# Jackie-Chou/MC-CNN-python

Measured on AMD Instinct MI355X. Metric: Mdisparities/s (HxWxD / s) end-to-end match.py timed region, images resident in HBM, higher is better.
Workload: dtype f32; 1 GPU; cfg2: 750x500 synthetic stereo pair, D=256, one pair per GPU; weights=converted reference checkpoint

## Files before the change

### mc-cnn-python_amd/csrc/cost_volume.hip

```cpp
#include "common.h"

namespace mccnn {

constexpr int CV_TW = 64;
constexpr int CV_DT = 64;
constexpr int CV_C = 64;
#ifndef CVM_WAVES_PER_SIMD
#define CVM_WAVES_PER_SIMD 6
#endif
constexpr int CV_LD = 68;

template <bool PIXEL_MAJOR>
__global__ __launch_bounds__(256) void cost_volume_exact_kernel(const float *__restrict__ fl,
                                                                const float *__restrict__ fr, int H, int W, int D,
                                                                float *__restrict__ lcv, float *__restrict__ rcv, int Dp)
{
    __shared__ __attribute__((aligned(16))) float sR[(CV_TW + CV_DT - 1) * CV_LD];
    __shared__ __attribute__((aligned(16))) float sL[CV_TW * CV_LD];
    const int w0 = blockIdx.x * CV_TW, h = blockIdx.y, d0 = blockIdx.z * CV_DT;
    if (w0 + CV_TW - 1 < d0) return;
    const int tid = threadIdx.x;
    const size_t rowbase = (size_t)h * W;
    for (int i = tid; i < CV_TW * 16; i += 256) {
        const int px = i >> 4, c4 = i & 15;
        float4 v = make_float4(0.f, 0.f, 0.f, 0.f);
        if (w0 + px < W) v = *reinterpret_cast<const float4 *>(fl + (rowbase + w0 + px) * CV_C + c4 * 4);
        *reinterpret_cast<float4 *>(&sL[px * CV_LD + c4 * 4]) = v;
    }
    const int xr0 = w0 - d0 - (CV_DT - 1);
    for (int i = tid; i < (CV_TW + CV_DT - 1) * 16; i += 256) {
        const int r = i >> 4, c4 = i & 15;
        const int x = xr0 + r;
        float4 v = make_float4(0.f, 0.f, 0.f, 0.f);
        if (x >= 0 && x < W) v = *reinterpret_cast<const float4 *>(fr + (rowbase + x) * CV_C + c4 * 4);
        *reinterpret_cast<float4 *>(&sR[r * CV_LD + c4 * 4]) = v;
    }
    __syncthreads();

    const int wl = tid & 63, dq = tid >> 6;
    const int w = w0 + wl;
    float a[CV_C];
#pragma unroll
    for (int c4 = 0; c4 < 16; ++c4) {
        const float4 v = *reinterpret_cast<const float4 *>(&sL[wl * CV_LD + c4 * 4]);
        a[c4 * 4 + 0] = v.x; a[c4 * 4 + 1] = v.y; a[c4 * 4 + 2] = v.z; a[c4 * 4 + 3] = v.w;
    }
    const size_t plane = (size_t)H * W;
    constexpr int TP = 65;
    float *const sT = sL;
    if (PIXEL_MAJOR) __syncthreads();
    for (int k = 0; k < 16; ++k) {
        const int d = d0 + dq * 16 + k;
        if (d >= D) break;
        const int r = wl + (CV_DT - 1) - (dq * 16 + k);
        if (w < W && w >= d) {
            const float *b = &sR[r * CV_LD];
            float acc[8];
#pragma unroll
            for (int i = 0; i < 8; ++i) {
                const float4 b0 = *reinterpret_cast<const float4 *>(b + i * 8);
                const float4 b1 = *reinterpret_cast<const float4 *>(b + i * 8 + 4);
                const float p0 = a[i * 8 + 0] * b0.x, p1 = a[i * 8 + 1] * b0.y, p2 = a[i * 8 + 2] * b0.z,
                            p3 = a[i * 8 + 3] * b0.w, p4 = a[i * 8 + 4] * b1.x, p5 = a[i * 8 + 5] * b1.y,
                            p6 = a[i * 8 + 6] * b1.z, p7 = a[i * 8 + 7] * b1.w;
                if (i == 0) {
                    acc[0] = p0; acc[1] = p1; acc[2] = p2; acc[3] = p3;
                    acc[4] = p4; acc[5] = p5; acc[6] = p6; acc[7] = p7;
                } else {
                    acc[0] += p0; acc[1] += p1; acc[2] += p2; acc[3] += p3;
                    acc[4] += p4; acc[5] += p5; acc[6] += p6; acc[7] += p7;
                }
            }
            float s = ((acc[0] + acc[1]) + (acc[2] + acc[3])) + ((acc[4] + acc[5]) + (acc[6] + acc[7]));
            s = 0.f + s;
            s = -1.f * s;
            if (PIXEL_MAJOR) {
                sT[wl * TP + dq * 16 + k] = s;
            } else {
                lcv[(size_t)d * plane + rowbase + w] = s;
                rcv[(size_t)d * plane + rowbase + (w - d)] = s;
            }
        }
    }
    if (PIXEL_MAJOR) {
        __syncthreads();
        const int nd = min(CV_DT, D - d0);
        const int dl = tid & 63;
        for (int px = tid >> 6; px < CV_TW; px += 4) {
            const int ww = w0 + px, d = d0 + dl;
            if (ww < W && dl < nd && ww >= d) lcv[(rowbase + ww) * (size_t)Dp + d] = sT[px * TP + dl];
        }
        for (int xi = tid >> 6; xi < CV_TW + CV_DT - 1; xi += 4) {
            const int x = xr0 + xi, d = d0 + dl, px = x + d - w0;
            if (x >= 0 && dl < nd && px >= 0 && px < CV_TW && w0 + px < W)
                rcv[(rowbase + x) * (size_t)Dp + d] = sT[px * TP + dl];
        }
    }
}

constexpr int CVP_TW = 63;
#ifndef CVP_ABL
#define CVP_ABL 0
#endif
__device__ __forceinline__ bool cvp_never(int D) { return D == 12345; }
__global__ __launch_bounds__(256, 3) void cost_volume_exact_pairs_kernel(const float *__restrict__ fl,
                                                                         const float *__restrict__ fr, int H, int W, int D,
                                                                         float *__restrict__ lcv, float *__restrict__ rcv,
                                                                         int Dp)
{
    constexpr int RING = 128;
    __shared__ __attribute__((aligned(16))) float sR[RING * CV_LD];
    __shared__ __attribute__((aligned(16))) float sL[CV_TW * CV_LD];
    const int w0 = (int)blockIdx.x * CVP_TW - 1, h = blockIdx.y;
    const int tid = threadIdx.x;
    const size_t rowbase = (size_t)h * W;
    for (int i = tid; i < CV_TW * 16; i += 256) {
        const int px = i >> 4, c4 = i & 15;
        float4 v = make_float4(0.f, 0.f, 0.f, 0.f);
        if (w0 + px >= 0 && w0 + px < W) v = *reinterpret_cast<const float4 *>(fl + (rowbase + w0 + px) * CV_C + c4 * 4);
        *reinterpret_cast<float4 *>(&sL[px * CV_LD + c4 * 4]) = v;
    }
    for (int i = tid; i < (CV_TW + CV_DT - 1) * 16; i += 256) {
        const int x = w0 - (CV_DT - 1) + (i >> 4), c4 = i & 15;
        float4 v = make_float4(0.f, 0.f, 0.f, 0.f);
        if (x >= 0 && x < W) v = *reinterpret_cast<const float4 *>(fr + (rowbase + x) * CV_C + c4 * 4);
        *reinterpret_cast<float4 *>(&sR[(x & (RING - 1)) * CV_LD + c4 * 4]) = v;
    }
    __syncthreads();

    const int wl = tid & 63, dq = tid >> 6;
    const int w = w0 + wl;
    float a[CV_C];
#pragma unroll
    for (int c4 = 0; c4 < 16; ++c4) {
        const float4 v = *reinterpret_cast<const float4 *>(&sL[wl * CV_LD + c4 * 4]);
        a[c4 * 4 + 0] = v.x; a[c4 * 4 + 1] = v.y; a[c4 * 4 + 2] = v.z; a[c4 * 4 + 3] = v.w;
    }
    constexpr int TP = CV_LD;
    float *const sT = sL;
    __syncthreads();
#pragma unroll 1
    for (int d0 = 0; d0 < D && w0 + CV_TW - 1 >= d0; d0 += CV_DT) {
        const bool more = d0 + CV_DT < D && w0 + CV_TW - 1 >= d0 + CV_DT;
        float4 nx[4];
#pragma unroll
        for (int q = 0; q < 4; ++q) {
            const int i = tid + q * 256, x = w0 - d0 - (2 * CV_DT - 1) + (i >> 4), c4 = i & 15;
            nx[q] = make_float4(0.f, 0.f, 0.f, 0.f);
            if (more && x >= 0 && x < W) nx[q] = *reinterpret_cast<const float4 *>(fr + (rowbase + x) * CV_C + c4 * 4);
        }
#pragma unroll 1
        for (int kk = 0; kk < (((CVP_ABL & 1) && !cvp_never(D)) ? 0 : 8); ++kk) {
            const int dloc = dq * 16 + 2 * kk;
            const int r = (w - d0 - dloc) & (RING - 1);
            const float *b = &sR[r * CV_LD];
            float acc[8], acn[8];
            float4 n0 = *reinterpret_cast<const float4 *>(b), n1 = *reinterpret_cast<const float4 *>(b + 4);
#pragma unroll
            for (int i = 0; i < 8; ++i) {
                const float bv[8] = {n0.x, n0.y, n0.z, n0.w, n1.x, n1.y, n1.z, n1.w};
                if (i < 7) {
                    n0 = *reinterpret_cast<const float4 *>(b + (i + 1) * 8);
                    n1 = *reinterpret_cast<const float4 *>(b + (i + 1) * 8 + 4);
                }
#pragma unroll
                for (int j = 0; j < 8; j += 4) {
                    if (i == 0) {
                        asm volatile("v_mul_f32 %0, %8, %12\n\tv_mul_f32 %1, %9, %13\n\tv_mul_f32 %2, %10, %14\n\tv_mul_f32 %3, %11, %15\n\t"
                                     "v_mul_f32_dpp %4, %12, %8 wave_shr:1 row_mask:0xf bank_mask:0xf bound_ctrl:1\n\t"
                                     "v_mul_f32_dpp %5, %13, %9 wave_shr:1 row_mask:0xf bank_mask:0xf bound_ctrl:1\n\t"
                                     "v_mul_f32_dpp %6, %14, %10 wave_shr:1 row_mask:0xf bank_mask:0xf bound_ctrl:1\n\t"
                                     "v_mul_f32_dpp %7, %15, %11 wave_shr:1 row_mask:0xf bank_mask:0xf bound_ctrl:1"
                                     : "=&v"(acc[j]), "=&v"(acc[j + 1]), "=&v"(acc[j + 2]), "=&v"(acc[j + 3]),
                                       "=&v"(acn[j]), "=&v"(acn[j + 1]), "=&v"(acn[j + 2]), "=&v"(acn[j + 3])
                                     : "v"(a[j]), "v"(a[j + 1]), "v"(a[j + 2]), "v"(a[j + 3]),
                                       "v"(bv[j]), "v"(bv[j + 1]), "v"(bv[j + 2]), "v"(bv[j + 3]));
                    } else {
                        float t0, t1, t2, t3;
                        asm volatile("v_mul_f32 %8, %12, %16\n\tv_mul_f32 %9, %13, %17\n\tv_mul_f32 %10, %14, %18\n\tv_mul_f32 %11, %15, %19\n\t"
                                     "v_add_f32 %0, %0, %8\n\tv_add_f32 %1, %1, %9\n\tv_add_f32 %2, %2, %10\n\tv_add_f32 %3, %3, %11\n\t"
                                     "v_mul_f32_dpp %8, %16, %12 wave_shr:1 row_mask:0xf bank_mask:0xf bound_ctrl:1\n\t"
                                     "v_mul_f32_dpp %9, %17, %13 wave_shr:1 row_mask:0xf bank_mask:0xf bound_ctrl:1\n\t"
                                     "v_mul_f32_dpp %10, %18, %14 wave_shr:1 row_mask:0xf bank_mask:0xf bound_ctrl:1\n\t"
                                     "v_mul_f32_dpp %11, %19, %15 wave_shr:1 row_mask:0xf bank_mask:0xf bound_ctrl:1\n\t"
                                     "v_add_f32 %4, %4, %8\n\tv_add_f32 %5, %5, %9\n\tv_add_f32 %6, %6, %10\n\tv_add_f32 %7, %7, %11"
                                     : "+v"(acc[j]), "+v"(acc[j + 1]), "+v"(acc[j + 2]), "+v"(acc[j + 3]),
                                       "+v"(acn[j]), "+v"(acn[j + 1]), "+v"(acn[j + 2]), "+v"(acn[j + 3]),
                                       "=&v"(t0), "=&v"(t1), "=&v"(t2), "=&v"(t3)
                                     : "v"(a[i * 8 + j]), "v"(a[i * 8 + j + 1]), "v"(a[i * 8 + j + 2]), "v"(a[i * 8 + j + 3]),
                                       "v"(bv[j]), "v"(bv[j + 1]), "v"(bv[j + 2]), "v"(bv[j + 3]));
                    }
                }
                __builtin_amdgcn_sched_barrier(0);
            }
            float s = ((acc[0] + acc[1]) + (acc[2] + acc[3])) + ((acc[4] + acc[5]) + (acc[6] + acc[7]));
            float sn = ((acn[0] + acn[1]) + (acn[2] + acn[3])) + ((acn[4] + acn[5]) + (acn[6] + acn[7]));
            s = 0.f + s;
            sn = 0.f + sn;
            s = -1.f * s;
            sn = -1.f * sn;
            const int d = d0 + dloc;
            if (wl >= 1 && w < W) {
                if (d < D && w >= d) sT[wl * TP + dloc] = s;
                if (d + 1 < D && w >= d + 1) sT[wl * TP + dloc + 1] = sn;
            }
        }
        __syncthreads();
#pragma unroll
        for (int q = 0; q < 4; ++q) {
            const int i = tid + q * 256, x = w0 - d0 - (2 * CV_DT - 1) + (i >> 4), c4 = i & 15;
            if (more) *reinterpret_cast<float4 *>(&sR[(x & (RING - 1)) * CV_LD + c4 * 4]) = nx[q];
        }
        const int nd = ((CVP_ABL & 2) && !cvp_never(D)) ? 0 : min(CV_DT, D - d0);
        const int xr0 = w0 - d0 - (CV_DT - 1);
        const int q4 = (tid & 15) * 4, sub = tid >> 4;
        for (int px = 1 + sub; px < CV_TW; px += 16) {
            const int ww = w0 + px, d = d0 + q4;
            if (ww >= W || q4 >= nd || ww < d) continue;
            const float4 v = *reinterpret_cast<const float4 *>(&sT[px * TP + q4]);
            float *dst = lcv + (rowbase + ww) * (size_t)Dp + d;
            if (q4 + 3 < nd && ww >= d + 3) {
                *reinterpret_cast<float4 *>(dst) = v;
            } else {
                const float e[4] = {v.x, v.y, v.z, v.w};
#pragma unroll
                for (int j = 0; j < 4; ++j)
                    if (q4 + j < nd && ww >= d + j) dst[j] = e[j];
            }
        }
        for (int xi = sub; xi < CV_TW + CV_DT - 1; xi += 16) {
            const int x = xr0 + xi, d = d0 + q4, px = x + d - w0;
            if (x < 0 || q4 >= nd || px + 3 < 1 || px >= CV_TW) continue;
            float *dst = rcv + (rowbase + x) * (size_t)Dp + d;
            if (q4 + 3 < nd && px >= 1 && px + 3 < CV_TW && w0 + px + 3 < W) {
                float4 v;
                v.x = sT[px * TP + q4];
                v.y = sT[(px + 1) * TP + q4 + 1];
                v.z = sT[(px + 2) * TP + q4 + 2];
                v.w = sT[(px + 3) * TP + q4 + 3];
                *reinterpret_cast<float4 *>(dst) = v;
            } else {
#pragma unroll
                for (int j = 0; j < 4; ++j)
                    if (q4 + j < nd && px + j >= 1 && px + j < CV_TW && w0 + px + j < W) dst[j] = sT[(px + j) * TP + q4 + j];
            }
        }
        __syncthreads();
    }
}

using f32x16 = __attribute__((ext_vector_type(16))) float;
typedef _Float16 cv_h8 __attribute__((ext_vector_type(8)));
typedef _Float16 cv_h4 __attribute__((ext_vector_type(4)));
constexpr int CVM_SP = 144;
constexpr int CVM_TP = 68;

__device__ __forceinline__ void cv_split4(const float4 v, cv_h4 &hi, cv_h4 &lo)
{
    const float x[4] = {__builtin_amdgcn_fmed3f(v.x * 1024.f, -65504.f, 65504.f),
                        __builtin_amdgcn_fmed3f(v.y * 1024.f, -65504.f, 65504.f),
                        __builtin_amdgcn_fmed3f(v.z * 1024.f, -65504.f, 65504.f),
                        __builtin_amdgcn_fmed3f(v.w * 1024.f, -65504.f, 65504.f)};
#pragma unroll
    for (int j = 0; j < 4; ++j) {
        const _Float16 h = (_Float16)x[j];
        hi[j] = h;
        lo[j] = (_Float16)(x[j] - (float)h);
    }
}

template <bool PIXEL_MAJOR>
__global__ __launch_bounds__(256, CVM_WAVES_PER_SIMD) void cost_volume_mfma_kernel(
    const float *__restrict__ fl, const float *__restrict__ fr, int H, int W, int D, float *__restrict__ lcv,
    float *__restrict__ rcv, int nwt, int nbands, int total, int Dp)
{
    constexpr int LDS_BYTES = (2 * 64 * CVM_SP > 64 * CVM_TP * 4) ? 2 * 64 * CVM_SP : 64 * CVM_TP * 4;
    __shared__ __attribute__((aligned(16))) char lds[LDS_BYTES];
    char *oL = lds, *oR = lds + 64 * CVM_SP;
    float *sT = reinterpret_cast<float *>(lds);
    int id;
    {
        const int b = blockIdx.x, qq = total >> 3, r = total & 7, xc = b & 7;
        id = (xc < r ? xc * (qq + 1) : r * (qq + 1) + (xc - r) * qq) + (b >> 3);
    }
    const int wt = id % nwt, band = (id / nwt) % nbands;
    const int h = id / (nwt * nbands);
    const int w0 = wt * 64;
    const int x0 = w0 - band * 64;
    if (x0 + 63 < 0) return;
    if (w0 - x0 - 63 >= D) return;
    const int tid = threadIdx.x;
    const size_t rowbase = (size_t)h * W;
    float4 vl[2][2], vr[2][2];
#pragma unroll
    for (int hf = 0; hf < 2; ++hf)
#pragma unroll
        for (int j = 0; j < 2; ++j) {
            const int p = j * 256 + tid, px = p >> 3, c4 = hf * 8 + (p & 7);
            vl[hf][j] = make_float4(0.f, 0.f, 0.f, 0.f);
            vr[hf][j] = make_float4(0.f, 0.f, 0.f, 0.f);
            if (w0 + px < W) vl[hf][j] = *reinterpret_cast<const float4 *>(fl + (rowbase + w0 + px) * CV_C + c4 * 4);
            const int x = x0 + px;
            if (x >= 0 && x < W) vr[hf][j] = *reinterpret_cast<const float4 *>(fr + (rowbase + x) * CV_C + c4 * 4);
        }
    const int wave = tid >> 6, lane = tid & 63;
    const int wr = (wave >> 1) * 32, wc = (wave & 1) * 32;
    f32x16 acc, acc2;
#pragma unroll
    for (int i = 0; i < 16; ++i) acc[i] = 0.f, acc2[i] = 0.f;
    const char *pa = oL + (wr + (lane & 31)) * CVM_SP + 16 * (lane >> 5);
    const char *pb = oR + (wc + (lane & 31)) * CVM_SP + 16 * (lane >> 5);
#pragma unroll
    for (int hf = 0; hf < 2; ++hf) {
        if (hf) __syncthreads();
#pragma unroll
        for (int j = 0; j < 2; ++j) {
            const int p = j * 256 + tid, px = p >> 3, c = p & 7;
            const int off = px * CVM_SP + (c >> 2) * 64 + (c & 3) * 8;
            cv_h4 hh, ll;
            cv_split4(vl[hf][j], hh, ll);
            *reinterpret_cast<cv_h4 *>(oL + off) = hh;
            *reinterpret_cast<cv_h4 *>(oL + off + 32) = ll;
            cv_split4(vr[hf][j], hh, ll);
            *reinterpret_cast<cv_h4 *>(oR + off) = hh;
            *reinterpret_cast<cv_h4 *>(oR + off + 32) = ll;
        }
        __syncthreads();
#pragma unroll
        for (int q = 0; q < 2; ++q) {
            const cv_h8 a_hi = *reinterpret_cast<const cv_h8 *>(pa + q * 64);
            const cv_h8 a_lo = *reinterpret_cast<const cv_h8 *>(pa + q * 64 + 32);
            const cv_h8 b_hi = *reinterpret_cast<const cv_h8 *>(pb + q * 64);
            const cv_h8 b_lo = *reinterpret_cast<const cv_h8 *>(pb + q * 64 + 32);
            acc2 = __builtin_amdgcn_mfma_f32_32x32x16_f16(a_lo, b_hi, acc2, 0, 0, 0);
            acc = __builtin_amdgcn_mfma_f32_32x32x16_f16(a_hi, b_hi, acc, 0, 0, 0);
            acc2 = __builtin_amdgcn_mfma_f32_32x32x16_f16(a_hi, b_lo, acc2, 0, 0, 0);
        }
    }
    __syncthreads();
    if (PIXEL_MAJOR) {
        constexpr int TP = 65;
#pragma unroll
        for (int rg = 0; rg < 16; ++rg) {
            const int row = wr + (rg & 3) + 8 * (rg >> 2) + 4 * (lane >> 5);
            const int col = wc + (lane & 31);
            sT[row * TP + col] = (acc[rg] + acc2[rg]) * (-1.f / 1048576.f);
        }
        __syncthreads();
        const int dbase = w0 - x0;
        for (int r = wave; r < 64; r += 4) {
            const int w = w0 + r, d = dbase + r - lane;
            if (w < W && d >= 0 && d < D && w >= d) lcv[(rowbase + w) * (size_t)Dp + d] = sT[r * TP + lane];
        }
        for (int c = wave; c < 64; c += 4) {
            const int x = x0 + c, d = dbase + lane - c;
            if (x >= 0 && w0 + lane < W && d >= 0 && d < D) rcv[(rowbase + x) * (size_t)Dp + d] = sT[lane * TP + c];
        }
        return;
    }
#pragma unroll
    for (int rg = 0; rg < 16; ++rg) {
        const int row = wr + (rg & 3) + 8 * (rg >> 2) + 4 * (lane >> 5);
        const int col = wc + (lane & 31);
        sT[((row - col) & 63) * CVM_TP + row] = (acc[rg] + acc2[rg]) * (-1.f / 1048576.f);
    }
    __syncthreads();
    const size_t plane = (size_t)H * W;
    const int dbase = w0 - x0;
    typedef float f4u __attribute__((ext_vector_type(4), aligned(4)));
    const int q = lane & 15, sub = lane >> 4;
    for (int rgp = wave; rgp < 16; rgp += 4) {
        const int row = rgp * 4 + sub;
        const int wl = 4 * q;
        const float4 t = *reinterpret_cast<const float4 *>(&sT[row * CVM_TP + wl]);
        const float v[4] = {t.x, t.y, t.z, t.w};
        const int w = w0 + wl;
        if (wl >= row || wl + 3 < row) {
            const int dd = wl >= row ? row : row - 64;
            const int d = dbase + dd;
            if (d < 0 || d >= D || w >= W) continue;
            float *pl = lcv + (size_t)d * plane + rowbase + w;
            float *pr = rcv + (size_t)d * plane + rowbase + (w - d);
            if (w + 3 < W) {
                f4u o;
                o[0] = v[0]; o[1] = v[1]; o[2] = v[2]; o[3] = v[3];
                *reinterpret_cast<f4u *>(pl) = o;
                *reinterpret_cast<f4u *>(pr) = o;
            } else {
#pragma unroll
                for (int j = 0; j < 4; ++j)
                    if (w + j < W) {
                        pl[j] = v[j];
                        pr[j] = v[j];
                    }
            }
        }
    }
    {
        const int row = tid >> 2, j = tid & 3;
        const int c = (row & ~3) + j;
        const int d = dbase + (c >= row ? row : row - 64);
        const int w = w0 + c;
        if ((row & 3) != 0 && d >= 0 && d < D && w < W) {
            const float v = sT[row * CVM_TP + c];
            lcv[(size_t)d * plane + rowbase + w] = v;
            rcv[(size_t)d * plane + rowbase + (w - d)] = v;
        }
    }
}

__global__ __launch_bounds__(64) void cost_volume_fill_kernel(float *__restrict__ lcv, float *__restrict__ rcv, int D,
                                                              int H, int W)
{
    __shared__ float tile[64 * 65];
    const int lane = threadIdx.x;
    const int d = D - 1 - blockIdx.y;
    const int h0 = blockIdx.x * 64;
    const int h = min(h0 + lane, H - 1);
    const int nrows = min(64, H - h0);
    if (blockIdx.z == 0) {
        float *L = lcv + ((size_t)d * H + h) * W;
        float x1 = L[d], x2 = L[d + 1], x3 = L[d + 2];
        for (int wtop = d - 1; wtop >= 0; wtop -= 64) {
            const int cnt = min(64, wtop + 1);
            for (int j = 0; j < cnt; ++j) {
                float s = 0.f - x1;
                s = s - x2;
                s = s - x3;
                const float v = -(s / 3.f);
                tile[lane * 65 + j] = v;
                x3 = x2; x2 = x1; x1 = v;
            }
            __syncthreads();
            if (lane < cnt)
                for (int r = 0; r < nrows; ++r)
                    lcv[((size_t)d * H + h0 + r) * W + (wtop - lane)] = tile[r * 65 + lane];
            __syncthreads();
        }
    } else {
        float *Rr = rcv + ((size_t)d * H + h) * W;
        float x1 = Rr[W - d - 3], x2 = Rr[W - d - 2], x3 = Rr[W - d - 1];
        for (int wbot = W - d; wbot < W; wbot += 64) {
            const int cnt = min(64, W - wbot);
            for (int j = 0; j < cnt; ++j) {
                float s = 0.f - x1;
                s = s - x2;
                s = s - x3;
                const float v = -(s / 3.f);
                tile[lane * 65 + j] = v;
                x1 = x2; x2 = x3; x3 = v;
            }
            __syncthreads();
            if (lane < cnt)
                for (int r = 0; r < nrows; ++r)
                    rcv[((size_t)d * H + h0 + r) * W + (wbot + lane)] = tile[r * 65 + lane];
            __syncthreads();
        }
    }
}

typedef uint32_t cv_u32x4 __attribute__((ext_vector_type(4)));
template <int NG>
__global__ __launch_bounds__(64) void cost_volume_fill_hwd_kernel(float *__restrict__ lcv, float *__restrict__ rcv, int D,
                                                                  int Dp, int H, int W)
{
    constexpr int PF = 8;
    constexpr int kDrop = 0x7ffffff0;
    const int lane = threadIdx.x, h = blockIdx.x;
    const bool left = blockIdx.y == 0;
    float *row = (left ? lcv : rcv) + (size_t)h * W * Dp;
    const __amdgpu_buffer_rsrc_t rs = __builtin_amdgcn_make_buffer_rsrc(row, 0, (int)((size_t)W * Dp * 4), 0x00020000);
    const unsigned pix = (unsigned)Dp * 4u;
    const int c_first = left ? D + 1 : max(W - D - 2, 0), nsteps = left ? D + 2 : W - c_first;
    auto col = [&](int t) { return left ? c_first - t : c_first + t; };
    int dbase[NG], voff[NG];
    float x1[NG][4], x2[NG][4], x3[NG][4];
#pragma unroll
    for (int g = 0; g < NG; ++g) {
        dbase[g] = g * 256 + lane * 4;
        voff[g] = dbase[g] < Dp ? dbase[g] * 4 : kDrop;
#pragma unroll
        for (int i = 0; i < 4; ++i) x1[g][i] = x2[g][i] = x3[g][i] = 0.f;
    }
    cv_u32x4 buf[PF][NG];
    auto issue = [&](int slot, int t) {
        const unsigned so = (unsigned)col(min(t, nsteps - 1)) * pix;
#pragma unroll
        for (int g = 0; g < NG; ++g) buf[slot][g] = __builtin_amdgcn_raw_buffer_load_b128(rs, voff[g], so, 0);
    };
#pragma unroll
    for (int k = 0; k < PF; ++k) issue(k, k);
    for (int t0 = 0; t0 < nsteps; t0 += PF) {
#pragma unroll
        for (int k = 0; k < PF; ++k) {
            const int t = t0 + k;
            if (t >= nsteps) continue;
            const int c = col(t);
#pragma unroll
            for (int g = 0; g < NG; ++g) {
                const cv_u32x4 u = buf[k][g];
                const float v[4] = {__uint_as_float(u.x), __uint_as_float(u.y), __uint_as_float(u.z), __uint_as_float(u.w)};
                cv_u32x4 o;
                bool any = false;
#pragma unroll
                for (int i = 0; i < 4; ++i) {
                    const int d = dbase[g] + i;
                    const bool stored = left ? c >= d : c < W - d;
                    float s = 0.f - x1[g][i];
                    s = s - x2[g][i];
                    s = s - x3[g][i];
                    const float val = stored ? v[i] : -(s / 3.f);
                    any |= !stored && d < D;
                    if (left) { x3[g][i] = x2[g][i]; x2[g][i] = x1[g][i]; x1[g][i] = val; }
                    else      { x1[g][i] = x2[g][i]; x2[g][i] = x3[g][i]; x3[g][i] = val; }
                    o[i] = __float_as_uint(val);
                }
                buffer_store_b128<0>(o, rs, any ? voff[g] : kDrop, (unsigned)c * pix);
            }
            issue(k, t + PF);
        }
    }
}


__global__ __launch_bounds__(64) void cost_volume_fill_hwd_lanes_kernel(float *__restrict__ lcv, float *__restrict__ rcv,
                                                                        int D, int Dp, int H, int W)
{
    constexpr int PF = 16;
    constexpr int kDrop = 0x7ffffff0;
    const int lane = threadIdx.x, h = blockIdx.x;
    const bool left = blockIdx.y == 0;
    const int d = (int)blockIdx.z * 64 + lane;
    const int dmax = min((int)blockIdx.z * 64 + 63, D - 1);
    if ((int)blockIdx.z * 64 >= D) return;
    float *row = (left ? lcv : rcv) + (size_t)h * W * Dp;
    const __amdgpu_buffer_rsrc_t rs = __builtin_amdgcn_make_buffer_rsrc(row, 0, (int)((size_t)W * Dp * 4), 0x00020000);
    const unsigned pix = (unsigned)Dp * 4u;
    const int c_first = left ? dmax + 2 : max(W - dmax - 3, 0), nsteps = left ? c_first + 1 : W - c_first;
    auto col = [&](int t) { return left ? c_first - t : c_first + t; };
    const int voff = d < Dp ? d * 4 : kDrop;
    const int sto = d < D ? voff : kDrop;
    float x1 = 0.f, x2 = 0.f, x3 = 0.f;
    float buf[PF];
    const int dmin = (int)blockIdx.z * 64;
    const int nA = min(nsteps, left ? c_first - dmin + 1 : (W - dmin) - c_first);
    auto issue = [&](int slot, int t) {
        const int c = col(min(t, nA - 1));
        buf[slot] = __uint_as_float(__builtin_amdgcn_raw_buffer_load_b32(rs, voff, (unsigned)c * pix, 0));
    };
    auto third = [](float s) {
        const float zh = 0.3333333432674407958984375f;
        const float q = s * zh;
        const float r = __builtin_fmaf(-3.0f, q, s);
        const float q2 = __builtin_fmaf(r, zh, q);
        return (__builtin_fabsf(s) < __builtin_inff() && s != 0.f) ? q2 : s;
    };
    auto step = [&](int c, bool stored, float have) {
        float s = 0.f - x1;
        s = s - x2;
        s = s - x3;
        const float val = stored ? have : -third(s);
        if (left) { x3 = x2; x2 = x1; x1 = val; }
        else      { x1 = x2; x2 = x3; x3 = val; }
        __builtin_amdgcn_raw_buffer_store_b32(__float_as_uint(val), rs, stored ? kDrop : sto, (unsigned)c * pix, 0);
    };
    if (nA > 0) {
#pragma unroll
        for (int k = 0; k < PF; ++k) issue(k, k);
        for (int t0 = 0; t0 < nA; t0 += PF) {
#pragma unroll
            for (int k = 0; k < PF; ++k) {
                const int t = t0 + k;
                if (t < nA) {
                    const int c = col(t);
                    step(c, left ? c >= d : c < W - d, buf[k]);
                }
                issue(k, t + PF);
            }
        }
    }
    for (int t = max(nA, 0); t < nsteps; ++t) step(col(t), false, 0.f);
}

int launch_cost_volume_fill(float *lcv, float *rcv, int D, int H, int W, hipStream_t s, const char *what)
{
    if (D > 1)
        hipLaunchKernelGGL(cost_volume_fill_kernel, dim3(cdiv(H, 64), D - 1, 2), dim3(64), 0, s, lcv, rcv, D, H, W);
    return check_launch(what);
}

int launch_cost_volume_fill_hwd(float *lcv_hwd, float *rcv_hwd, int D, int Dp, int H, int W, hipStream_t s, const char *what)
{
    if (D > 1) {
#ifdef CV_FILL_FOUR_PER_LANE
        if (Dp <= 256)
            hipLaunchKernelGGL(cost_volume_fill_hwd_kernel<1>, dim3(H, 2), dim3(64), 0, s, lcv_hwd, rcv_hwd, D, Dp, H, W);
        else
            hipLaunchKernelGGL(cost_volume_fill_hwd_kernel<2>, dim3(H, 2), dim3(64), 0, s, lcv_hwd, rcv_hwd, D, Dp, H, W);
#else
        hipLaunchKernelGGL(cost_volume_fill_hwd_lanes_kernel, dim3(H, 2, cdiv(D, 64)), dim3(64), 0, s, lcv_hwd, rcv_hwd, D, Dp,
                           H, W);
#endif
    }
    return check_launch(what);
}

}

extern "C" int mccnn_cost_volume(const float *fl, const float *fr, int H, int W, int C, int D, float *lcv, float *rcv,
                                 int mode, mccnn_stream_t stream)
{
    using namespace mccnn;
    MCCNN_REQUIRE(fl && fr && lcv && rcv, MCCNN_E_INVALID, "mccnn_cost_volume: null pointer");
    MCCNN_REQUIRE(H > 0 && W > 0 && D > 0, MCCNN_E_INVALID, "mccnn_cost_volume: non-positive size");
    MCCNN_REQUIRE(C == CV_C, MCCNN_E_UNSUPPORTED, "mccnn_cost_volume: C=%d, kernels are built for 64 channels", C);
    MCCNN_REQUIRE(D <= W - 2, MCCNN_E_UNSUPPORTED,
                  "mccnn_cost_volume: D=%d needs W >= D+2 (the reference's border recurrence pf:106 is degenerate "
                  "beyond that), W=%d", D, W);
    hipStream_t s = (hipStream_t)stream;
    const dim3 block(256);
    if (mode == MCCNN_CV_EXACT) {
        const dim3 grid(cdiv(W, CV_TW), H, cdiv(D, CV_DT));
        hipLaunchKernelGGL(cost_volume_exact_kernel<false>, grid, block, 0, s, fl, fr, H, W, D, lcv, rcv, 0);
    } else if (mode == MCCNN_CV_MFMA) {
        const int nwt = cdiv(W, 64), nbands = cdiv(D + 63, 64) + 1;
        const long total = (long)nwt * nbands * H;
        MCCNN_REQUIRE(total <= 0x7fffffffL, MCCNN_E_UNSUPPORTED, "mccnn_cost_volume: %ld tiles exceed the grid", total);
        hipLaunchKernelGGL(cost_volume_mfma_kernel<false>, dim3((unsigned)total), block, 0, s, fl, fr, H, W, D, lcv, rcv, nwt,
                           nbands, (int)total, 0);
    } else {
        MCCNN_REQUIRE(false, MCCNN_E_INVALID, "mccnn_cost_volume: unknown mode %d", mode);
    }
    int rc = check_launch("mccnn_cost_volume");
    if (rc) return rc;
    return launch_cost_volume_fill(lcv, rcv, D, H, W, s, "mccnn_cost_volume(fill)");
}

extern "C" int mccnn_cost_volume_hwd(const float *fl, const float *fr, int H, int W, int C, int D, float *lcv_hwd,
                                     float *rcv_hwd, int mode, mccnn_stream_t stream)
{
    using namespace mccnn;
    MCCNN_REQUIRE(fl && fr && lcv_hwd && rcv_hwd, MCCNN_E_INVALID, "mccnn_cost_volume_hwd: null pointer");
    MCCNN_REQUIRE(H > 0 && W > 0 && D > 0, MCCNN_E_INVALID, "mccnn_cost_volume_hwd: non-positive size");
    MCCNN_REQUIRE(C == CV_C, MCCNN_E_UNSUPPORTED, "mccnn_cost_volume_hwd: C=%d, kernels are built for 64 channels", C);
    MCCNN_REQUIRE(D <= W - 2, MCCNN_E_UNSUPPORTED,
                  "mccnn_cost_volume_hwd: D=%d needs W >= D+2 (the reference's border recurrence pf:106 is degenerate "
                  "beyond that), W=%d", D, W);
    MCCNN_REQUIRE(mode == MCCNN_CV_EXACT || mode == MCCNN_CV_MFMA, MCCNN_E_INVALID, "mccnn_cost_volume_hwd: unknown mode %d",
                  mode);
#ifdef CV_FILL_FOUR_PER_LANE
    constexpr int kMaxD = 512;
#else
    constexpr int kMaxD = 1024;
#endif
    MCCNN_REQUIRE(D <= kMaxD, MCCNN_E_UNSUPPORTED, "mccnn_cost_volume_hwd: D=%d > %d", D, kMaxD);
    const int Dp = mccnn_hwd_pitch(D);
    MCCNN_REQUIRE((size_t)W * Dp * 4 < ((size_t)1 << 31), MCCNN_E_UNSUPPORTED,
                  "mccnn_cost_volume_hwd: a %d x %d row exceeds a buffer descriptor's reach", W, D);
    hipStream_t s = (hipStream_t)stream;
    if (mode == MCCNN_CV_MFMA) {
        const int nwt = cdiv(W, 64), nbands = cdiv(D + 63, 64) + 1;
        const long total = (long)nwt * nbands * H;
        MCCNN_REQUIRE(total <= 0x7fffffffL, MCCNN_E_UNSUPPORTED, "mccnn_cost_volume_hwd: %ld tiles exceed the grid", total);
        hipLaunchKernelGGL(cost_volume_mfma_kernel<true>, dim3((unsigned)total), dim3(256), 0, s, fl, fr, H, W, D, lcv_hwd,
                           rcv_hwd, nwt, nbands, (int)total, Dp);
    } else {
#ifdef CV_HWD_TILE_KERNEL
        const dim3 grid(cdiv(W, CV_TW), H, cdiv(D, CV_DT));
        hipLaunchKernelGGL(cost_volume_exact_kernel<true>, grid, dim3(256), 0, s, fl, fr, H, W, D, lcv_hwd, rcv_hwd, Dp);
#else
        const dim3 grid(cdiv(W, CVP_TW), H, 1);
        hipLaunchKernelGGL(cost_volume_exact_pairs_kernel, grid, dim3(256), 0, s, fl, fr, H, W, D, lcv_hwd, rcv_hwd, Dp);
#endif
    }
    int rc = check_launch("mccnn_cost_volume_hwd");
    if (rc) return rc;
    return launch_cost_volume_fill_hwd(lcv_hwd, rcv_hwd, D, Dp, H, W, s, "mccnn_cost_volume_hwd(fill)");
}

extern "C" int mccnn_cost_volume_fill(float *lcv, float *rcv, int D, int H, int W, int pixel_major, mccnn_stream_t stream)
{
    using namespace mccnn;
    MCCNN_REQUIRE(lcv && rcv, MCCNN_E_INVALID, "mccnn_cost_volume_fill: null pointer");
    MCCNN_REQUIRE(H > 0 && W > 0 && D > 0, MCCNN_E_INVALID, "mccnn_cost_volume_fill: non-positive size");
    MCCNN_REQUIRE(D <= W - 2, MCCNN_E_UNSUPPORTED, "mccnn_cost_volume_fill: D=%d needs W >= D+2, W=%d", D, W);
    if (!pixel_major) return launch_cost_volume_fill(lcv, rcv, D, H, W, (hipStream_t)stream, "mccnn_cost_volume_fill");
    const int Dp = mccnn_hwd_pitch(D);
    MCCNN_REQUIRE(D <= 1024, MCCNN_E_UNSUPPORTED, "mccnn_cost_volume_fill: D=%d > 1024", D);
    MCCNN_REQUIRE((size_t)W * Dp * 4 < ((size_t)1 << 31), MCCNN_E_UNSUPPORTED,
                  "mccnn_cost_volume_fill: a %d x %d row exceeds a buffer descriptor's reach", W, D);
    return launch_cost_volume_fill_hwd(lcv, rcv, D, Dp, H, W, (hipStream_t)stream, "mccnn_cost_volume_fill");
}
```

Measured before the change: 11580 Mdisparities/s.

## Streamline cost-volume pair kernel stores with nontemporal writes and precomputed masks

Rewrites the store phase of the pairs cost-volume kernel. Per-thread row limits and 32-bit byte offsets are computed once outside the disparity loop. The data-dependent per-pixel loops become unrolled, branch-light full float4 stores, with a bitmask-driven fallback for ragged edges. Output writes become nontemporal by default, and the feature loads are clamped instead of predicated so they can all be issued before the LDS writes. This is meant to cut address arithmetic, divergence and cache pollution on the write-bound cost-volume output. The cost is loads from clamped, duplicated addresses, plus 32-bit offsets that could overflow on larger volumes.

Result: no change. 11780 Mdisparities/s (median of 6 runs) (+1.8%).

```diff
diff --git a/mc-cnn-python_amd/csrc/cost_volume.hip b/mc-cnn-python_amd/csrc/cost_volume.hip
--- a/mc-cnn-python_amd/csrc/cost_volume.hip
+++ b/mc-cnn-python_amd/csrc/cost_volume.hip
@@ -103,6 +103,18 @@
 #define CVP_ABL 0
 #endif
 __device__ __forceinline__ bool cvp_never(int D) { return D == 12345; }
+#ifndef CVP_NT
+#define CVP_NT 1
+#endif
+typedef float cv_f4 __attribute__((ext_vector_type(4)));
+__device__ __forceinline__ void cvp_store16(char *dst, cv_f4 v)
+{
+#if CVP_NT
+    __builtin_nontemporal_store(v, reinterpret_cast<cv_f4 *>(dst));
+#else
+    *reinterpret_cast<cv_f4 *>(dst) = v;
+#endif
+}
 __global__ __launch_bounds__(256, 3) void cost_volume_exact_pairs_kernel(const float *__restrict__ fl,
                                                                          const float *__restrict__ fr, int H, int W, int D,
                                                                          float *__restrict__ lcv, float *__restrict__ rcv,
@@ -114,17 +126,28 @@
     const int w0 = (int)blockIdx.x * CVP_TW - 1, h = blockIdx.y;
     const int tid = threadIdx.x;
     const size_t rowbase = (size_t)h * W;
-    for (int i = tid; i < CV_TW * 16; i += 256) {
-        const int px = i >> 4, c4 = i & 15;
-        float4 v = make_float4(0.f, 0.f, 0.f, 0.f);
-        if (w0 + px >= 0 && w0 + px < W) v = *reinterpret_cast<const float4 *>(fl + (rowbase + w0 + px) * CV_C + c4 * 4);
-        *reinterpret_cast<float4 *>(&sL[px * CV_LD + c4 * 4]) = v;
-    }
-    for (int i = tid; i < (CV_TW + CV_DT - 1) * 16; i += 256) {
-        const int x = w0 - (CV_DT - 1) + (i >> 4), c4 = i & 15;
-        float4 v = make_float4(0.f, 0.f, 0.f, 0.f);
-        if (x >= 0 && x < W) v = *reinterpret_cast<const float4 *>(fr + (rowbase + x) * CV_C + c4 * 4);
-        *reinterpret_cast<float4 *>(&sR[(x & (RING - 1)) * CV_LD + c4 * 4]) = v;
+    {
+        cv_f4 pl[4], pr[8];
+#pragma unroll
+        for (int q = 0; q < 4; ++q) {
+            const int i = tid + q * 256, x = w0 + (i >> 4), c4 = i & 15;
+            pl[q] = *reinterpret_cast<const cv_f4 *>(fl + (rowbase + min(max(x, 0), W - 1)) * CV_C + c4 * 4);
+        }
+#pragma unroll
+        for (int q = 0; q < 8; ++q) {
+            const int i = tid + q * 256, x = w0 - (CV_DT - 1) + (i >> 4), c4 = i & 15;
+            pr[q] = *reinterpret_cast<const cv_f4 *>(fr + (rowbase + min(max(x, 0), W - 1)) * CV_C + c4 * 4);
+        }
+#pragma unroll
+        for (int q = 0; q < 4; ++q) {
+            const int i = tid + q * 256, px = i >> 4, c4 = i & 15;
+            *reinterpret_cast<cv_f4 *>(&sL[px * CV_LD + c4 * 4]) = pl[q];
+        }
+#pragma unroll
+        for (int q = 0; q < 8; ++q) {
+            const int i = tid + q * 256, x = w0 - (CV_DT - 1) + (i >> 4), c4 = i & 15;
+            *reinterpret_cast<cv_f4 *>(&sR[(x & (RING - 1)) * CV_LD + c4 * 4]) = pr[q];
+        }
     }
     __syncthreads();
 
@@ -138,16 +161,33 @@
     }
     constexpr int TP = CV_LD;
     float *const sT = sL;
+    const int q4 = (tid & 15) * 4, sub = tid >> 4;
+    const int dlast = ((CVP_ABL & 2) && !cvp_never(D)) ? -1 : D - 1;
+    int lim_l[4], lim_r[8];
+    unsigned whole_r = 0;
+#pragma unroll
+    for (int k = 0; k < 4; ++k) {
+        const int px = 1 + sub + 16 * k, ww = w0 + px;
+        lim_l[k] = (px < CV_TW && ww < W) ? min(ww, dlast) : -1;
+    }
+#pragma unroll
+    for (int k = 0; k < 8; ++k) {
+        const int px = sub + 16 * k - (CV_DT - 1) + q4;
+        lim_r[k] = (px + 3 >= 1 && px < CV_TW) ? min(w0 + px, dlast) : -1;
+        whole_r |= (px >= 1 && px + 3 < CV_TW && w0 + px + 3 < W) ? 1u << k : 0u;
+    }
+    const int Dp4 = Dp * 4;
+    const unsigned vo_l = (unsigned)((w0 + 1 + sub) * Dp + q4) * 4u;
+    const unsigned vo_r = (unsigned)((w0 - (CV_DT - 1) + sub) * Dp + q4) * 4u;
+    char *const lrow = reinterpret_cast<char *>(lcv + rowbase * Dp), *const rrow = reinterpret_cast<char *>(rcv + rowbase * Dp);
     __syncthreads();
 #pragma unroll 1
     for (int d0 = 0; d0 < D && w0 + CV_TW - 1 >= d0; d0 += CV_DT) {
-        const bool more = d0 + CV_DT < D && w0 + CV_TW - 1 >= d0 + CV_DT;
-        float4 nx[4];
+        cv_f4 nx[4];
 #pragma unroll
         for (int q = 0; q < 4; ++q) {
             const int i = tid + q * 256, x = w0 - d0 - (2 * CV_DT - 1) + (i >> 4), c4 = i & 15;
-            nx[q] = make_float4(0.f, 0.f, 0.f, 0.f);
-            if (more && x >= 0 && x < W) nx[q] = *reinterpret_cast<const float4 *>(fr + (rowbase + x) * CV_C + c4 * 4);
+            nx[q] = *reinterpret_cast<const cv_f4 *>(fr + (rowbase + min(max(x, 0), W - 1)) * CV_C + c4 * 4);
         }
 #pragma unroll 1
         for (int kk = 0; kk < (((CVP_ABL & 1) && !cvp_never(D)) ? 0 : 8); ++kk) {
@@ -209,41 +249,61 @@
 #pragma unroll
         for (int q = 0; q < 4; ++q) {
             const int i = tid + q * 256, x = w0 - d0 - (2 * CV_DT - 1) + (i >> 4), c4 = i & 15;
-            if (more) *reinterpret_cast<float4 *>(&sR[(x & (RING - 1)) * CV_LD + c4 * 4]) = nx[q];
-        }
-        const int nd = ((CVP_ABL & 2) && !cvp_never(D)) ? 0 : min(CV_DT, D - d0);
-        const int xr0 = w0 - d0 - (CV_DT - 1);
-        const int q4 = (tid & 15) * 4, sub = tid >> 4;
-        for (int px = 1 + sub; px < CV_TW; px += 16) {
-            const int ww = w0 + px, d = d0 + q4;
-            if (ww >= W || q4 >= nd || ww < d) continue;
-            const float4 v = *reinterpret_cast<const float4 *>(&sT[px * TP + q4]);
-            float *dst = lcv + (rowbase + ww) * (size_t)Dp + d;
-            if (q4 + 3 < nd && ww >= d + 3) {
-                *reinterpret_cast<float4 *>(dst) = v;
-            } else {
-                const float e[4] = {v.x, v.y, v.z, v.w};
-#pragma unroll
-                for (int j = 0; j < 4; ++j)
-                    if (q4 + j < nd && ww >= d + j) dst[j] = e[j];
-            }
-        }
-        for (int xi = sub; xi < CV_TW + CV_DT - 1; xi += 16) {
-            const int x = xr0 + xi, d = d0 + q4, px = x + d - w0;
-            if (x < 0 || q4 >= nd || px + 3 < 1 || px >= CV_TW) continue;
-            float *dst = rcv + (rowbase + x) * (size_t)Dp + d;
-            if (q4 + 3 < nd && px >= 1 && px + 3 < CV_TW && w0 + px + 3 < W) {
-                float4 v;
-                v.x = sT[px * TP + q4];
-                v.y = sT[(px + 1) * TP + q4 + 1];
-                v.z = sT[(px + 2) * TP + q4 + 2];
-                v.w = sT[(px + 3) * TP + q4 + 3];
-                *reinterpret_cast<float4 *>(dst) = v;
-            } else {
-#pragma unroll
-                for (int j = 0; j < 4; ++j)
-                    if (q4 + j < nd && px + j >= 1 && px + j < CV_TW && w0 + px + j < W) dst[j] = sT[(px + j) * TP + q4 + j];
-            }
+            *reinterpret_cast<cv_f4 *>(&sR[(x & (RING - 1)) * CV_LD + c4 * 4]) = nx[q];
+        }
+        const int d = d0 + q4;
+        unsigned rag = 0;
+        {
+            cv_f4 v[4];
+#pragma unroll
+            for (int k = 0; k < 4; ++k)
+                v[k] = *reinterpret_cast<const cv_f4 *>(&sT[min(1 + sub + 16 * k, CV_TW - 1) * TP + q4]);
+#pragma unroll
+            for (int k = 0; k < 4; ++k) asm volatile("" : "+v"(v[k]));
+#pragma unroll
+            for (int k = 0; k < 4; ++k) {
+                const bool full = d + 3 <= lim_l[k];
+                if (__builtin_expect(full, 1)) cvp_store16(lrow + (vo_l + (unsigned)(d0 * 4 + k * 16 * Dp4)), v[k]);
+                rag |= (d <= lim_l[k] && !full) ? 1u << k : 0u;
+            }
+        }
+        {
+#pragma unroll
+            for (int k0 = 0; k0 < 8; k0 += 4) {
+                cv_f4 v[4];
+#pragma unroll
+                for (int k = 0; k < 4; ++k) {
+                    const int pc = min(max(sub + 16 * (k0 + k) - (CV_DT - 1) + q4, 0), CV_TW - 4);
+                    v[k].x = sT[pc * TP + q4];
+                    v[k].y = sT[(pc + 1) * TP + q4 + 1];
+                    v[k].z = sT[(pc + 2) * TP + q4 + 2];
+                    v[k].w = sT[(pc + 3) * TP + q4 + 3];
+                }
+#pragma unroll
+                for (int k = 0; k < 4; ++k) asm volatile("" : "+v"(v[k]));
+#pragma unroll
+                for (int k = 0; k < 4; ++k) {
+                    const bool some = d <= lim_r[k0 + k];
+                    const bool full = some && ((whole_r >> (k0 + k)) & 1) && d + 3 <= dlast;
+                    if (__builtin_expect(full, 1))
+                        cvp_store16(rrow + (vo_r + (unsigned)(d0 * 4 + ((k0 + k) * 16 - d0) * Dp4)), v[k]);
+                    rag |= (some && !full) ? 16u << (k0 + k) : 0u;
+                }
+            }
+        }
+        for (unsigned m = rag & 15u; m; m &= m - 1) {
+            const int k = __builtin_ctz(m), px = 1 + sub + 16 * k, lim = min(w0 + px, dlast);
+            float *dst = reinterpret_cast<float *>(lrow + (vo_l + (unsigned)(d0 * 4 + k * 16 * Dp4)));
+#pragma unroll
+            for (int j = 0; j < 4; ++j)
+                if (d + j <= lim) dst[j] = sT[px * TP + q4 + j];
+        }
+        for (unsigned m = rag >> 4; m; m &= m - 1) {
+            const int k = __builtin_ctz(m), px = sub + 16 * k - (CV_DT - 1) + q4;
+            float *dst = reinterpret_cast<float *>(rrow + (vo_r + (unsigned)(d0 * 4 + (k * 16 - d0) * Dp4)));
+#pragma unroll
+            for (int j = 0; j < 4; ++j)
+                if (d + j <= dlast && px + j >= 1 && px + j < CV_TW && w0 + px + j < W) dst[j] = sT[(px + j) * TP + q4 + j];
         }
         __syncthreads();
     }
```
